# mir-group/nequip

Hardware: NVIDIA H100
Metric: atom-steps/sec (energy+forces) (higher is better)
Workload: dtype f32

## Files before the change

### nequip_b200/csrc/nqb_gemm.cu

```cuda
#include <cuda_runtime.h>
#include <stdint.h>

#include "../../include/nqb.h"
#include "nqb_tc.cuh"

namespace {

constexpr int TM = 128;
constexpr int TN = 128;
constexpr int KC = 32;
constexpr int MW = 64;
constexpr int NWG = TM / MW;
constexpr int DEPTH = 2;
constexpr int RAW = DEPTH + 1;
constexpr int NLO = 2;
constexpr int BSLOTS = 4;
constexpr int SEG = 320 / KC;
constexpr int NTHREADS = NWG * 128;
constexpr int BLOCK_FLOATS = 2 * TN * KC;

struct GemmDesc {
  int64_t a_off, c_off, b_off, rs_off;
  int64_t lda, ldc, K, N;
  int64_t kchunks, ntiles, tile0, flags;
};

struct Smem {
  float b[BSLOTS][BLOCK_FLOATS];
  float araw[NWG][RAW][MW * KC];
  float alo[NWG][NLO][MW * KC];
  uint64_t b_full[BSLOTS], b_empty[BSLOTS];
};

__device__ __forceinline__ const GemmDesc* find_desc(const GemmDesc* d, int nd, int q) {
  int i = 0;
  while (i + 1 < nd && d[i + 1].tile0 <= q) ++i;
  return d + i;
}

struct Sched {
  int q, q_step, nq_total;
  int64_t m_start, m_step;
  __device__ Sched(int b, int G, int T, const int32_t* tile_ctas, int sched_ctas) {
    nq_total = T;
    if (tile_ctas != nullptr && G == sched_ctas) {
      q = T; q_step = T; m_start = 0; m_step = 1;
      for (int t = 0; t < T; ++t) {
        const int c0 = tile_ctas[2 * t], n = tile_ctas[2 * t + 1];
        if (b >= c0 && b < c0 + n) { q = t; m_start = b - c0; m_step = n; break; }
      }
    } else if (T <= G) {
      const int R = G / T;
      q = (b < T * R) ? (b % T) : T;
      q_step = T;
      m_start = b / T;
      m_step = R;
    } else {
      q = b; q_step = G; m_start = 0; m_step = 1;
    }
  }
};

struct WorkQ {
  const GemmDesc* d;
  int nt, kchunks, K, ncols;
  bool resident;
};
__device__ __forceinline__ void decode_q(const GemmDesc* descs, int ndesc, int q, WorkQ& w) {
  w.d = find_desc(descs, ndesc, q);
  w.nt = q - (int)w.d->tile0;
  w.kchunks = (int)w.d->kchunks;
  w.K = (int)w.d->K;
  w.ncols = min(TN, (int)w.d->N - w.nt * TN);
  w.resident = w.kchunks <= BSLOTS;
}

__device__ __forceinline__ void bar_wg(int wg) { asm volatile("bar.sync %0, 128;" ::"r"(1 + wg) : "memory"); }

__global__ void __launch_bounds__(NTHREADS, 1)
k_gemm3x(const GemmDesc* __restrict__ descs, int ndesc, int ntiles_total, const int32_t* __restrict__ tile_ctas,
         int sched_ctas, const float* __restrict__ a_base, const float* __restrict__ b_base, float* __restrict__ c_base,
         const float* __restrict__ rs_base, int64_t rs_ld, int64_t M) {
  extern __shared__ __align__(1024) uint8_t smem_raw[];
  Smem& S = *reinterpret_cast<Smem*>(smem_raw);
  const int tid = threadIdx.x, wg = tid >> 7, warp = (tid >> 5) & 3, lane = tid & 31;
  const int64_t mtiles = (M + TM - 1) / TM;

  if (tid == 0) {
    for (int s = 0; s < BSLOTS; ++s) { mbar_init(&S.b_full[s], 1); mbar_init(&S.b_empty[s], NWG * 4); }
    fence_barrier_init();
  }
  __syncthreads();
  const Sched sch(blockIdx.x, gridDim.x, ntiles_total, tile_ctas, sched_ctas);

  const int r8 = lane & 7, kq = lane >> 3;
  const int my_off = (2 * warp) * (KC / 4 * 32) + kq * 32 + r8 * 4;
  int pq = sch.q, ph_ = 0, pnh = 1, pK = 0;
  int64_t pmt = sch.m_start, plda = 0;
  const float* pA = nullptr;
  bool pvalid = pq < sch.nq_total && sch.m_start < mtiles;
  auto open_q = [&]() {
    WorkQ w;
    decode_q(descs, ndesc, pq, w);
    pA = a_base + w.d->a_off;
    plda = w.d->lda;
    pK = w.K;
    pnh = w.kchunks;
  };
  if (pvalid) open_q();
  uint32_t n_issued = 0;
  auto issue = [&]() {
    if (pvalid) {
      float* dst = S.araw[wg][n_issued % RAW] + my_off;
#pragma unroll
      for (int g = 0; g < 2; ++g) {
        const int64_t m = pmt * TM + wg * MW + warp * 16 + g * 8 + r8;
#pragma unroll
        for (int kh = 0; kh < 2; ++kh) {
          const int k = ph_ * KC + (kh * 4 + kq) * 4;
          const bool in = m < M && k < pK;
          const int64_t off = in ? m * plda + k : 0;
          cp_async16(dst + g * (KC / 4 * 32) + kh * 128, pA + off, in ? 16u : 0u);
        }
      }
      if (++ph_ == pnh) {
        ph_ = 0;
        pmt += sch.m_step;
        if (pmt >= mtiles) {
          pmt = sch.m_start;
          pq += sch.q_step;
          pvalid = pq < sch.nq_total;
          if (pvalid) open_q();
        }
      }
    }
    ++n_issued;
    cp_async_commit();
  };
#pragma unroll 1
  for (int j = 0; j < DEPTH; ++j) issue();

  uint32_t bused = 0, bpar_ld = 0;
  auto load_slot = [&](int slot, const float* src, uint32_t bytes) {
    if ((bused >> slot) & 1) mbar_wait(&S.b_empty[slot], ((bpar_ld >> slot) & 1) ^ 1);
    mbar_expect_tx(&S.b_full[slot], 2 * bytes);
    bulk_g2s(S.b[slot], src, bytes, &S.b_full[slot]);
    bulk_g2s(S.b[slot] + TN * KC, src + TN * KC, bytes, &S.b_full[slot]);
    bused |= 1u << slot;
    bpar_ld ^= 1u << slot;
  };
  uint32_t bpar = 0;

  constexpr uint32_t SBO = (KC / 4) * 128, LBO = 128;
  constexpr uint32_t A_STAGE = (MW * KC * sizeof(float)) >> 4;
  constexpr uint32_t B_SLOT = (BLOCK_FLOATS * sizeof(float)) >> 4, B_LO = (TN * KC * sizeof(float)) >> 4;
  const uint64_t dR0 = make_desc(smem_u32(S.araw[wg][0]), LBO, SBO);
  const uint64_t dL0 = make_desc(smem_u32(S.alo[wg][0]), LBO, SBO);
  const uint64_t dB0 = make_desc(smem_u32(S.b[0]), LBO, SBO);
  const int r0 = warp * 16 + (lane >> 2), c0 = 2 * (lane & 3);
  float hh[64], xx[64], acc[64];
  uint32_t i = 0;

  for (int q = sch.q; q < sch.nq_total; q += sch.q_step) {
    WorkQ w;
    decode_q(descs, ndesc, q, w);
    if (sch.m_start >= mtiles) continue;
    const GemmDesc* d = w.d;
    const int nseg = (w.kchunks + SEG - 1) / SEG;
    const int64_t nmt = (mtiles - 1 - sch.m_start) / sch.m_step + 1;
    const int64_t nload = w.resident ? w.kchunks : nmt * w.kchunks;
    const uint32_t bytes = (uint32_t)TN * KC * sizeof(float);
    const float* B = b_base + d->b_off + (int64_t)w.nt * w.kchunks * BLOCK_FLOATS;
    if (tid == 0)
      for (int64_t c = 0; c < min((int64_t)BSLOTS, nload); ++c) load_slot((int)c, B + (c % w.kchunks) * BLOCK_FLOATS, bytes);
    int64_t x = 0;
    const bool reduce = (d->flags & 5) != 0, skipz = (d->flags & 2) != 0;
    const int64_t ldc = d->ldc;
    float* C = c_base + d->c_off + (int64_t)w.nt * TN;
    bool first_mt = true;
    for (int64_t mt = sch.m_start; mt < mtiles; mt += sch.m_step) {
      for (int seg = 0; seg < nseg; ++seg) {
        const int h1 = min(w.kchunks, (seg + 1) * SEG);
        for (int h = seg * SEG; h < h1; ++h, ++i) {
          cp_async_wait<DEPTH - 1>();
          const float* raw = S.araw[wg][i % RAW] + my_off;
          float* lo = S.alo[wg][i % NLO] + my_off;
#pragma unroll
          for (int g = 0; g < 2; ++g)
#pragma unroll
            for (int kh = 0; kh < 2; ++kh) {
              const float4 t = *reinterpret_cast<const float4*>(raw + g * (KC / 4 * 32) + kh * 128);
              *reinterpret_cast<float4*>(lo + g * (KC / 4 * 32) + kh * 128) =
                  make_float4(tf32_lo(t.x), tf32_lo(t.y), tf32_lo(t.z), tf32_lo(t.w));
            }
          fence_proxy_async();
          bar_wg(wg);
          uint32_t slot;
          if (w.resident) {
            slot = h;
            if (first_mt) { mbar_wait(&S.b_full[slot], (bpar >> slot) & 1); bpar ^= 1u << slot; }
          } else {
            slot = (uint32_t)(x % BSLOTS);
            mbar_wait(&S.b_full[slot], (bpar >> slot) & 1);
            bpar ^= 1u << slot;
          }
          const uint64_t a_hi = dR0 + (uint64_t)((i % RAW) * A_STAGE), a_lo = dL0 + (uint64_t)((i % NLO) * A_STAGE);
          const uint64_t b_hi = dB0 + (uint64_t)(slot * B_SLOT), b_lo = b_hi + B_LO;
          const uint32_t fresh = (h == seg * SEG);
          wgmma_fence();
#pragma unroll
          for (int ks = 0; ks < KC / 8; ++ks) wgmma_tf32_m64n128(hh, a_hi + ks * 16, b_hi + ks * 16, !(fresh && ks == 0));
#pragma unroll
          for (int ks = 0; ks < KC / 8; ++ks) wgmma_tf32_m64n128(xx, a_lo + ks * 16, b_hi + ks * 16, !(fresh && ks == 0));
#pragma unroll
          for (int ks = 0; ks < KC / 8; ++ks) wgmma_tf32_m64n128(xx, a_hi + ks * 16, b_lo + ks * 16, 1u);
          wgmma_commit();
          wgmma_wait<0>();
          if (!w.resident) {
            if (lane == 0) mbar_arrive(&S.b_empty[slot]);
            if (tid == 0 && x + BSLOTS < nload) load_slot(slot, B + ((x + BSLOTS) % w.kchunks) * BLOCK_FLOATS, bytes);
            ++x;
          }
          issue();
        }
        if (seg + 1 < nseg) {
#pragma unroll
          for (int j = 0; j < 64; ++j) acc[j] = (seg == 0 ? 0.f : acc[j]) + (hh[j] + xx[j]);
        } else {
#pragma unroll
          for (int j = 0; j < 64; ++j) hh[j] = (seg == 0) ? hh[j] + xx[j] : acc[j] + (hh[j] + xx[j]);
        }
      }
      const int64_t m0 = mt * TM + wg * MW + r0;
#pragma unroll
      for (int half = 0; half < 2; ++half) {
        const int64_t m = m0 + half * 8;
        float rs = 1.0f;
        if (d->rs_off >= 0) rs = (m < M) ? __ldg(rs_base + d->rs_off * rs_ld + m) : 0.f;
        if (m >= M || (skipz && rs == 0.f)) continue;
        float* crow = C + m * ldc + c0;
#pragma unroll
        for (int j = 0; j < TN / 8; ++j) {
          if (j * 8 + c0 < w.ncols) {
            const float v0 = hh[4 * j + 2 * half] * rs, v1 = hh[4 * j + 2 * half + 1] * rs;
            if (reduce)
              asm volatile("red.global.add.v2.f32 [%0], {%1, %2};" ::"l"(crow + j * 8), "f"(v0), "f"(v1) : "memory");
            else
              *reinterpret_cast<float2*>(crow + j * 8) = make_float2(v0, v1);
          }
        }
      }
      first_mt = false;
    }
    if (w.resident && lane == 0)
      for (int c = 0; c < w.kchunks; ++c) mbar_arrive(&S.b_empty[c]);
  }
  cp_async_wait<0>();
}

__global__ void k_gemm_prepare(const float* __restrict__ B, int64_t ldb, int K, int N, int transposed, float scale,
                               float* __restrict__ out, int kchunks, int ntiles) {
  const int64_t total = (int64_t)ntiles * kchunks * TN * KC;
  for (int64_t idx = (int64_t)blockIdx.x * blockDim.x + threadIdx.x; idx < total; idx += (int64_t)gridDim.x * blockDim.x) {
    const int kk = (int)(idx % KC);
    const int nn = (int)((idx / KC) % TN);
    const int64_t blk = idx / (KC * TN);
    const int c = (int)(blk % kchunks), j = (int)(blk / kchunks);
    const int k = c * KC + kk, n = j * TN + nn;
    float v = 0.f;
    if (k < K && n < N) v = (transposed ? B[(int64_t)n * ldb + k] : B[(int64_t)k * ldb + n]) * scale;
    const float hi = tf32_rn(v), lo = v - hi;
    float* tile = out + blk * BLOCK_FLOATS;
    const int off = canon_off(nn, kk, KC / 4);
    tile[off] = hi;
    tile[TN * KC + off] = lo;
  }
}

}

extern "C" int nqb_set_error(const char* msg);
extern "C" void nqb_count_launch(void);

static int gemm_device() {
  int dev = 0;
  cudaGetDevice(&dev);
  return dev & 63;
}
static int gemm_sm_count() {
  static int n[64] = {0};
  const int dev = gemm_device();
  if (n[dev] == 0) {
    cudaDeviceGetAttribute(&n[dev], cudaDevAttrMultiProcessorCount, dev);
    if (n[dev] <= 0) n[dev] = 132;
  }
  return n[dev];
}

extern "C" int64_t nqb_gemm_prepared_floats(int K, int N) {
  const int64_t kchunks = (K + KC - 1) / KC, ntiles = (N + TN - 1) / TN;
  return kchunks * ntiles * BLOCK_FLOATS;
}

extern "C" int nqb_gemm_prepare(const float* B, int64_t ldb, int K, int N, int transposed, float scale, float* prepared,
                                nqb_stream_t st) {
  if (!B || !prepared) return nqb_set_error("nqb_gemm_prepare: null pointer");
  if (K <= 0 || N <= 0) return nqb_set_error("nqb_gemm_prepare: bad shape");
  const int kchunks = (K + KC - 1) / KC, ntiles = (N + TN - 1) / TN;
  const int64_t total = (int64_t)ntiles * kchunks * TN * KC;
  int blocks = (int)((total + 255) / 256);
  if (blocks > 4096) blocks = 4096;
  k_gemm_prepare<<<blocks, 256, 0, (cudaStream_t)st>>>(B, ldb, K, N, transposed, scale, prepared, kchunks, ntiles);
  nqb_count_launch();
  cudaError_t e = cudaGetLastError();
  if (e != cudaSuccess) return nqb_set_error(cudaGetErrorString(e));
  return 0;
}

extern "C" int nqb_gemm_grouped(const void* descs_dev, int ndesc, int ntiles_total, const int32_t* tile_ctas_dev,
                                int sched_ctas, const float* a_base, const float* prepared_base, float* c_base,
                                const float* rowscale_base, int64_t rs_ld, int64_t M, nqb_stream_t st) {
  if (ndesc <= 0 || ntiles_total <= 0) return nqb_set_error("nqb_gemm_grouped: empty problem list");
  if (M < 0) return nqb_set_error("nqb_gemm_grouped: negative M");
  if (M == 0) return 0;
  if (!descs_dev || !a_base || !prepared_base || !c_base) return nqb_set_error("nqb_gemm_grouped: null pointer");
  static bool attr_set[64] = {false};
  const int dev = gemm_device();
  if (!attr_set[dev]) {
    cudaError_t e = cudaFuncSetAttribute(k_gemm3x, cudaFuncAttributeMaxDynamicSharedMemorySize, (int)sizeof(Smem) + 1024);
    if (e != cudaSuccess) return nqb_set_error(cudaGetErrorString(e));
    attr_set[dev] = true;
  }
  const int64_t nwork = ((M + TM - 1) / TM) * (int64_t)ntiles_total;
  int grid = (int)(nwork < gemm_sm_count() ? nwork : gemm_sm_count());
  if (tile_ctas_dev != nullptr && sched_ctas > 0 && sched_ctas <= gemm_sm_count()) grid = sched_ctas;
  else tile_ctas_dev = nullptr;
  k_gemm3x<<<grid, NTHREADS, sizeof(Smem) + 1024, (cudaStream_t)st>>>((const GemmDesc*)descs_dev, ndesc, ntiles_total, tile_ctas_dev, sched_ctas, a_base,
                                                                 prepared_base, c_base, rowscale_base, rs_ld, M);
  nqb_count_launch();
  cudaError_t e = cudaGetLastError();
  if (e != cudaSuccess) return nqb_set_error(cudaGetErrorString(e));
  return 0;
}
```

### nequip_b200/csrc/nqb_tc.cuh

```cuda
#pragma once
#define NQB_TC_HELPERS 1
#include <cuda_runtime.h>
#include <stdint.h>

namespace {

__device__ __forceinline__ uint32_t smem_u32(const void* p) { return (uint32_t)__cvta_generic_to_shared(p); }

__device__ __forceinline__ void mbar_init(uint64_t* bar, uint32_t count) {
  asm volatile("mbarrier.init.shared::cta.b64 [%0], %1;" ::"r"(smem_u32(bar)), "r"(count));
}
__device__ __forceinline__ void mbar_arrive(uint64_t* bar) {
  asm volatile("mbarrier.arrive.shared::cta.b64 _, [%0];" ::"r"(smem_u32(bar)) : "memory");
}
__device__ __forceinline__ void mbar_expect_tx(uint64_t* bar, uint32_t bytes) {
  asm volatile("mbarrier.arrive.expect_tx.shared::cta.b64 _, [%0], %1;" ::"r"(smem_u32(bar)), "r"(bytes) : "memory");
}
__device__ __forceinline__ void mbar_wait(uint64_t* bar, uint32_t parity) {
  asm volatile(
      "{\n\t"
      ".reg .pred p;\n\t"
      "WAIT_%=:\n\t"
      "mbarrier.try_wait.parity.shared::cta.b64 p, [%0], %1;\n\t"
      "@p bra DONE_%=;\n\t"
      "bra WAIT_%=;\n\t"
      "DONE_%=:\n\t"
      "}" ::"r"(smem_u32(bar)), "r"(parity) : "memory");
}
__device__ __forceinline__ void fence_barrier_init() { asm volatile("fence.mbarrier_init.release.cluster;" ::: "memory"); }
__device__ __forceinline__ void fence_proxy_async() { asm volatile("fence.proxy.async.shared::cta;" ::: "memory"); }
__device__ __forceinline__ void bulk_g2s(void* dst, const void* src, uint32_t bytes, uint64_t* bar) {
  asm volatile("cp.async.bulk.shared::cluster.global.mbarrier::complete_tx::bytes [%0], [%1], %2, [%3];" ::"r"(smem_u32(dst)),
               "l"(src), "r"(bytes), "r"(smem_u32(bar))
               : "memory");
}

__device__ __forceinline__ float4 ldg_stream(const float* p) {
  float4 v;
  asm volatile("ld.global.nc.L1::no_allocate.v4.f32 {%0, %1, %2, %3}, [%4];" : "=f"(v.x), "=f"(v.y), "=f"(v.z), "=f"(v.w) : "l"(p));
  return v;
}
__device__ __forceinline__ void cp_async16(void* dst, const void* src, uint32_t src_bytes) {
  asm volatile("cp.async.cg.shared.global [%0], [%1], 16, %2;" ::"r"(smem_u32(dst)), "l"(src), "r"(src_bytes) : "memory");
}
__device__ __forceinline__ void cp_async_commit() { asm volatile("cp.async.commit_group;" ::: "memory"); }
template <int N>
__device__ __forceinline__ void cp_async_wait() { asm volatile("cp.async.wait_group %0;" ::"n"(N) : "memory"); }
__device__ __forceinline__ float tf32_rn(float a) {
  uint32_t r;
  asm("cvt.rna.tf32.f32 %0, %1;" : "=r"(r) : "f"(a));
  return __uint_as_float(r);
}
__device__ __forceinline__ float tf32_lo(float a) {
  const float hi = __uint_as_float(__float_as_uint(a) & 0xffffe000u);
  return tf32_rn(a - hi);
}
__device__ __forceinline__ void bulk_s2g(void* dst, const void* src, uint32_t bytes) {
  asm volatile("cp.async.bulk.global.shared::cta.bulk_group [%0], [%1], %2;" ::"l"(dst), "r"(smem_u32(src)), "r"(bytes)
               : "memory");
}
__device__ __forceinline__ void bulk_s2g_add(float* dst, const float* src, uint32_t bytes) {
  asm volatile("cp.reduce.async.bulk.global.shared::cta.bulk_group.add.f32 [%0], [%1], %2;" ::"l"(dst),
               "r"(smem_u32(src)), "r"(bytes)
               : "memory");
}
__device__ __forceinline__ void bulk_commit() { asm volatile("cp.async.bulk.commit_group;" ::: "memory"); }
__device__ __forceinline__ void bulk_wait_read0() { asm volatile("cp.async.bulk.wait_group.read 0;" ::: "memory"); }
__device__ __forceinline__ void bulk_wait_all() { asm volatile("cp.async.bulk.wait_group 0;" ::: "memory"); }
__device__ __forceinline__ uint64_t make_desc(uint32_t saddr, uint32_t lbo_bytes, uint32_t sbo_bytes) {
  uint64_t d = 0;
  d |= (uint64_t)((saddr >> 4) & 0x3FFF);
  d |= (uint64_t)((lbo_bytes >> 4) & 0x3FFF) << 16;
  d |= (uint64_t)((sbo_bytes >> 4) & 0x3FFF) << 32;
  return d;
}
__device__ __forceinline__ void wgmma_fence() { asm volatile("wgmma.fence.sync.aligned;" ::: "memory"); }
__device__ __forceinline__ void wgmma_commit() { asm volatile("wgmma.commit_group.sync.aligned;" ::: "memory"); }
template <int N>
__device__ __forceinline__ void wgmma_wait() { asm volatile("wgmma.wait_group.sync.aligned %0;" ::"n"(N) : "memory"); }
__device__ __forceinline__ void wgmma_tf32_m64n128(float* d, uint64_t desc_a, uint64_t desc_b, uint32_t accumulate) {
  asm volatile(
      "{\n\t"
      ".reg .pred p;\n\t"
      "setp.ne.b32 p, %66, 0;\n\t"
      "wgmma.mma_async.sync.aligned.m64n128k8.f32.tf32.tf32 "
      "{%0, %1, %2, %3, %4, %5, %6, %7, %8, %9, %10, %11, %12, %13, %14, %15, %16, %17, %18, %19, %20, %21, %22, %23, %24, %25, %26, %27, %28, %29, %30, %31, %32, %33, %34, %35, %36, %37, %38, %39, %40, %41, %42, %43, %44, %45, %46, %47, %48, %49, %50, %51, %52, %53, %54, %55, %56, %57, %58, %59, %60, %61, %62, %63}, "
      "%64, %65, p, 1, 1;\n\t"
      "}"
      : "+f"(d[0]), "+f"(d[1]), "+f"(d[2]), "+f"(d[3]), "+f"(d[4]), "+f"(d[5]), "+f"(d[6]), "+f"(d[7]),
        "+f"(d[8]), "+f"(d[9]), "+f"(d[10]), "+f"(d[11]), "+f"(d[12]), "+f"(d[13]), "+f"(d[14]), "+f"(d[15]),
        "+f"(d[16]), "+f"(d[17]), "+f"(d[18]), "+f"(d[19]), "+f"(d[20]), "+f"(d[21]), "+f"(d[22]), "+f"(d[23]),
        "+f"(d[24]), "+f"(d[25]), "+f"(d[26]), "+f"(d[27]), "+f"(d[28]), "+f"(d[29]), "+f"(d[30]), "+f"(d[31]),
        "+f"(d[32]), "+f"(d[33]), "+f"(d[34]), "+f"(d[35]), "+f"(d[36]), "+f"(d[37]), "+f"(d[38]), "+f"(d[39]),
        "+f"(d[40]), "+f"(d[41]), "+f"(d[42]), "+f"(d[43]), "+f"(d[44]), "+f"(d[45]), "+f"(d[46]), "+f"(d[47]),
        "+f"(d[48]), "+f"(d[49]), "+f"(d[50]), "+f"(d[51]), "+f"(d[52]), "+f"(d[53]), "+f"(d[54]), "+f"(d[55]),
        "+f"(d[56]), "+f"(d[57]), "+f"(d[58]), "+f"(d[59]), "+f"(d[60]), "+f"(d[61]), "+f"(d[62]), "+f"(d[63])
      : "l"(desc_a), "l"(desc_b), "r"(accumulate));
}

__device__ __forceinline__ void wgmma_tf32_m64n64(float* d, uint64_t desc_a, uint64_t desc_b, uint32_t accumulate) {
  asm volatile(
      "{\n\t"
      ".reg .pred p;\n\t"
      "setp.ne.b32 p, %34, 0;\n\t"
      "wgmma.mma_async.sync.aligned.m64n64k8.f32.tf32.tf32 "
      "{%0, %1, %2, %3, %4, %5, %6, %7, %8, %9, %10, %11, %12, %13, %14, %15, %16, %17, %18, %19, %20, %21, %22, %23, %24, %25, %26, %27, %28, %29, %30, %31}, "
      "%32, %33, p, 1, 1;\n\t"
      "}"
      : "+f"(d[0]), "+f"(d[1]), "+f"(d[2]), "+f"(d[3]), "+f"(d[4]), "+f"(d[5]), "+f"(d[6]), "+f"(d[7]),
        "+f"(d[8]), "+f"(d[9]), "+f"(d[10]), "+f"(d[11]), "+f"(d[12]), "+f"(d[13]), "+f"(d[14]), "+f"(d[15]),
        "+f"(d[16]), "+f"(d[17]), "+f"(d[18]), "+f"(d[19]), "+f"(d[20]), "+f"(d[21]), "+f"(d[22]), "+f"(d[23]),
        "+f"(d[24]), "+f"(d[25]), "+f"(d[26]), "+f"(d[27]), "+f"(d[28]), "+f"(d[29]), "+f"(d[30]), "+f"(d[31])
      : "l"(desc_a), "l"(desc_b), "r"(accumulate));
}

__device__ __forceinline__ float2 fma2_rn(float2 a, float2 b, float2 c) {
  return make_float2(__fmaf_rn(a.x, b.x, c.x), __fmaf_rn(a.y, b.y, c.y));
}
__device__ __forceinline__ float2 fmul2_rn(float2 a, float2 b) { return make_float2(__fmul_rn(a.x, b.x), __fmul_rn(a.y, b.y)); }

__device__ __forceinline__ float silu_f(float x) { return x / (1.0f + expf(-x)); }

__device__ __forceinline__ int canon_off(int row, int k, int kgroups) {
  return (row >> 3) * (kgroups * 32) + (k >> 2) * 32 + (row & 7) * 4 + (k & 3);
}


}
```

Before: 361,800.

## Warp-specialize 3xTF32 GEMM with producer warpgroup and register-sourced A fragments

Restructures the 3xTF32 WGMMA GEMM into a warp-specialized kernel. A dedicated producer warpgroup with fewer registers streams A tiles via cp.async with mbarrier completion and B tiles via bulk copies. The two consumer warpgroups get more registers, split A into hi/lo TF32 parts in registers, and issue register-sourced wgmma with one group in flight, so the lo-part smem round trip and the per-chunk wait are gone. Segment partial sums move to shared memory, and a named-barrier handoff staggers the two consumers. This adds barrier complexity and shared-memory pressure, with a risk of hangs if the parity bookkeeping is wrong.

Result: faster. 450,700 (median of 6 runs) (+24.6%).

```diff
diff --git a/nequip_b200/csrc/nqb_gemm.cu b/nequip_b200/csrc/nqb_gemm.cu
--- a/nequip_b200/csrc/nqb_gemm.cu
+++ b/nequip_b200/csrc/nqb_gemm.cu
@@ -11,13 +11,13 @@
 constexpr int KC = 32;
 constexpr int MW = 64;
 constexpr int NWG = TM / MW;
-constexpr int DEPTH = 2;
-constexpr int RAW = DEPTH + 1;
-constexpr int NLO = 2;
+constexpr int ASLOTS = 2;
 constexpr int BSLOTS = 4;
 constexpr int SEG = 320 / KC;
-constexpr int NTHREADS = NWG * 128;
+constexpr int NTHREADS = (NWG + 1) * 128;
 constexpr int BLOCK_FLOATS = 2 * TN * KC;
+constexpr int PRODUCER_REGS = 56, CONSUMER_REGS = 224;
+constexpr int BAR_TURN = 1;
 
 struct GemmDesc {
   int64_t a_off, c_off, b_off, rs_off;
@@ -27,9 +27,10 @@
 
 struct Smem {
   float b[BSLOTS][BLOCK_FLOATS];
-  float araw[NWG][RAW][MW * KC];
-  float alo[NWG][NLO][MW * KC];
+  float acc[NWG][MW * TN];
+  float a[NWG][ASLOTS][MW * KC];
   uint64_t b_full[BSLOTS], b_empty[BSLOTS];
+  uint64_t a_full[NWG][ASLOTS], a_empty[NWG][ASLOTS];
 };
 
 __device__ __forceinline__ const GemmDesc* find_desc(const GemmDesc* d, int nd, int q) {
@@ -75,163 +76,157 @@
   w.resident = w.kchunks <= BSLOTS;
 }
 
-__device__ __forceinline__ void bar_wg(int wg) { asm volatile("bar.sync %0, 128;" ::"r"(1 + wg) : "memory"); }
-
-__global__ void __launch_bounds__(NTHREADS, 1)
-k_gemm3x(const GemmDesc* __restrict__ descs, int ndesc, int ntiles_total, const int32_t* __restrict__ tile_ctas,
-         int sched_ctas, const float* __restrict__ a_base, const float* __restrict__ b_base, float* __restrict__ c_base,
-         const float* __restrict__ rs_base, int64_t rs_ld, int64_t M) {
-  extern __shared__ __align__(1024) uint8_t smem_raw[];
-  Smem& S = *reinterpret_cast<Smem*>(smem_raw);
-  const int tid = threadIdx.x, wg = tid >> 7, warp = (tid >> 5) & 3, lane = tid & 31;
-  const int64_t mtiles = (M + TM - 1) / TM;
-
-  if (tid == 0) {
-    for (int s = 0; s < BSLOTS; ++s) { mbar_init(&S.b_full[s], 1); mbar_init(&S.b_empty[s], NWG * 4); }
-    fence_barrier_init();
-  }
-  __syncthreads();
-  const Sched sch(blockIdx.x, gridDim.x, ntiles_total, tile_ctas, sched_ctas);
-
-  const int r8 = lane & 7, kq = lane >> 3;
-  const int my_off = (2 * warp) * (KC / 4 * 32) + kq * 32 + r8 * 4;
-  int pq = sch.q, ph_ = 0, pnh = 1, pK = 0;
-  int64_t pmt = sch.m_start, plda = 0;
-  const float* pA = nullptr;
-  bool pvalid = pq < sch.nq_total && sch.m_start < mtiles;
-  auto open_q = [&]() {
-    WorkQ w;
-    decode_q(descs, ndesc, pq, w);
-    pA = a_base + w.d->a_off;
-    plda = w.d->lda;
-    pK = w.K;
-    pnh = w.kchunks;
-  };
-  if (pvalid) open_q();
-  uint32_t n_issued = 0;
-  auto issue = [&]() {
-    if (pvalid) {
-      float* dst = S.araw[wg][n_issued % RAW] + my_off;
-#pragma unroll
-      for (int g = 0; g < 2; ++g) {
-        const int64_t m = pmt * TM + wg * MW + warp * 16 + g * 8 + r8;
-#pragma unroll
-        for (int kh = 0; kh < 2; ++kh) {
-          const int k = ph_ * KC + (kh * 4 + kq) * 4;
-          const bool in = m < M && k < pK;
-          const int64_t off = in ? m * plda + k : 0;
-          cp_async16(dst + g * (KC / 4 * 32) + kh * 128, pA + off, in ? 16u : 0u);
-        }
-      }
-      if (++ph_ == pnh) {
-        ph_ = 0;
-        pmt += sch.m_step;
-        if (pmt >= mtiles) {
-          pmt = sch.m_start;
-          pq += sch.q_step;
-          pvalid = pq < sch.nq_total;
-          if (pvalid) open_q();
-        }
-      }
-    }
-    ++n_issued;
-    cp_async_commit();
-  };
-#pragma unroll 1
-  for (int j = 0; j < DEPTH; ++j) issue();
-
-  uint32_t bused = 0, bpar_ld = 0;
-  auto load_slot = [&](int slot, const float* src, uint32_t bytes) {
-    if ((bused >> slot) & 1) mbar_wait(&S.b_empty[slot], ((bpar_ld >> slot) & 1) ^ 1);
-    mbar_expect_tx(&S.b_full[slot], 2 * bytes);
-    bulk_g2s(S.b[slot], src, bytes, &S.b_full[slot]);
-    bulk_g2s(S.b[slot] + TN * KC, src + TN * KC, bytes, &S.b_full[slot]);
-    bused |= 1u << slot;
-    bpar_ld ^= 1u << slot;
-  };
-  uint32_t bpar = 0;
-
-  constexpr uint32_t SBO = (KC / 4) * 128, LBO = 128;
-  constexpr uint32_t A_STAGE = (MW * KC * sizeof(float)) >> 4;
-  constexpr uint32_t B_SLOT = (BLOCK_FLOATS * sizeof(float)) >> 4, B_LO = (TN * KC * sizeof(float)) >> 4;
-  const uint64_t dR0 = make_desc(smem_u32(S.araw[wg][0]), LBO, SBO);
-  const uint64_t dL0 = make_desc(smem_u32(S.alo[wg][0]), LBO, SBO);
-  const uint64_t dB0 = make_desc(smem_u32(S.b[0]), LBO, SBO);
-  const int r0 = warp * 16 + (lane >> 2), c0 = 2 * (lane & 3);
-  float hh[64], xx[64], acc[64];
-  uint32_t i = 0;
-
-  for (int q = sch.q; q < sch.nq_total; q += sch.q_step) {
+__device__ __forceinline__ void produce_a(Smem& S, int c, int lane, const Sched& sch, const GemmDesc* descs, int ndesc,
+                                          const float* a_base, int64_t M, int64_t mtiles) {
+  const int p = lane & 7, r0 = lane >> 3;
+  uint32_t n = 0;
+  for (int q = sch.q; q < sch.nq_total && sch.m_start < mtiles; q += sch.q_step) {
     WorkQ w;
     decode_q(descs, ndesc, q, w);
-    if (sch.m_start >= mtiles) continue;
-    const GemmDesc* d = w.d;
-    const int nseg = (w.kchunks + SEG - 1) / SEG;
+    const float* A = a_base + w.d->a_off;
+    const int64_t lda = w.d->lda;
+    for (int64_t mt = sch.m_start; mt < mtiles; mt += sch.m_step) {
+      for (int h = 0; h < w.kchunks; ++h, ++n) {
+        const uint32_t s = n % ASLOTS;
+        if (n >= ASLOTS) mbar_wait(&S.a_empty[c][s], ((n / ASLOTS) - 1) & 1);
+        float* dst = S.a[c][s] + r0 * KC;
+        const int k = h * KC + 4 * p;
+        const bool kin = k < w.K;
+        int64_t m = mt * TM + c * MW + r0;
+#pragma unroll 4
+        for (int j = 0; j < MW / 4; ++j, m += 4) {
+          const bool in = kin && m < M;
+          cp_async16(dst + 4 * j * KC + 4 * (p ^ (r0 + 4 * (j & 1))), in ? A + m * lda + k : A, in ? 16u : 0u);
+        }
+        cp_async_mbar_arrive(&S.a_full[c][s]);
+      }
+    }
+  }
+  cp_async_wait<0>();
+}
+
+__device__ __forceinline__ void produce_b(Smem& S, const Sched& sch, const GemmDesc* descs, int ndesc,
+                                          const float* b_base, int64_t mtiles) {
+  uint32_t bused = 0, bpar_ld = 0;
+  constexpr uint32_t bytes = (uint32_t)TN * KC * sizeof(float);
+  for (int q = sch.q; q < sch.nq_total && sch.m_start < mtiles; q += sch.q_step) {
+    WorkQ w;
+    decode_q(descs, ndesc, q, w);
     const int64_t nmt = (mtiles - 1 - sch.m_start) / sch.m_step + 1;
     const int64_t nload = w.resident ? w.kchunks : nmt * w.kchunks;
-    const uint32_t bytes = (uint32_t)TN * KC * sizeof(float);
-    const float* B = b_base + d->b_off + (int64_t)w.nt * w.kchunks * BLOCK_FLOATS;
-    if (tid == 0)
-      for (int64_t c = 0; c < min((int64_t)BSLOTS, nload); ++c) load_slot((int)c, B + (c % w.kchunks) * BLOCK_FLOATS, bytes);
-    int64_t x = 0;
+    const float* B = b_base + w.d->b_off + (int64_t)w.nt * w.kchunks * BLOCK_FLOATS;
+    for (int64_t x = 0; x < nload; ++x) {
+      const int slot = (int)(x % BSLOTS);
+      if ((bused >> slot) & 1) mbar_wait(&S.b_empty[slot], ((bpar_ld >> slot) & 1) ^ 1);
+      const float* src = B + (x % w.kchunks) * BLOCK_FLOATS;
+      mbar_expect_tx(&S.b_full[slot], 2 * bytes);
+      bulk_g2s(S.b[slot], src, bytes, &S.b_full[slot]);
+      bulk_g2s(S.b[slot] + TN * KC, src + TN * KC, bytes, &S.b_full[slot]);
+      bused |= 1u << slot;
+      bpar_ld ^= 1u << slot;
+    }
+  }
+}
+
+__device__ __forceinline__ void consume(Smem& S, int c, int tid, const Sched& sch, const GemmDesc* descs, int ndesc,
+                                        float* c_base, const float* rs_base, int64_t rs_ld, int64_t M, int64_t mtiles) {
+  const int warp = (tid >> 5) & 3, lane = tid & 31, ltid = tid & 127;
+  const int g = lane >> 2, t = lane & 3;
+  const int r0 = warp * 16 + g, c0 = 2 * t;
+  const float* a_frag = S.a[c][0] + r0 * KC + t;
+  float* acc = S.acc[c] + ltid;
+
+  constexpr uint32_t SBO = (KC / 4) * 128, LBO = 128;
+  constexpr uint32_t B_SLOT = (BLOCK_FLOATS * sizeof(float)) >> 4, B_LO = (TN * KC * sizeof(float)) >> 4;
+  const uint64_t dB0 = make_desc(smem_u32(S.b[0]), LBO, SBO);
+  float hh[64], xx[64];
+  uint32_t ra0[32], ra1[32];
+  uint32_t na = 0;
+  uint32_t bpar = 0;
+  bool turn_owed = false;
+
+  for (int q = sch.q; q < sch.nq_total && sch.m_start < mtiles; q += sch.q_step) {
+    WorkQ w;
+    decode_q(descs, ndesc, q, w);
+    const GemmDesc* d = w.d;
+    const int kc = w.kchunks;
     const bool reduce = (d->flags & 5) != 0, skipz = (d->flags & 2) != 0;
     const int64_t ldc = d->ldc;
     float* C = c_base + d->c_off + (int64_t)w.nt * TN;
+    int64_t x = 0;
+    int held = -1;
     bool first_mt = true;
+    auto release_b = [&](int slot) {
+      if (lane == 0) mbar_arrive(&S.b_empty[slot]);
+    };
+    auto step = [&](uint32_t(&ra)[32], int h) {
+      const uint32_t s = na % ASLOTS;
+      mbar_wait(&S.a_full[c][s], (na / ASLOTS) & 1);
+      const float* src = a_frag + s * (MW * KC);
+#pragma unroll
+      for (int ks = 0; ks < KC / 8; ++ks)
+#pragma unroll
+        for (int e = 0; e < 4; ++e) {
+          const float v = src[(e & 1) * 8 * KC + 4 * ((2 * ks + (e >> 1)) ^ g)];
+          const float hi = __uint_as_float(__float_as_uint(v) & 0xffffe000u);
+          ra[4 * ks + e] = __float_as_uint(hi);
+          ra[16 + 4 * ks + e] = __float_as_uint(tf32_rn(v - hi));
+        }
+      __syncwarp();
+      if (lane == 0) mbar_arrive(&S.a_empty[c][s]);
+      ++na;
+      uint32_t slot;
+      if (w.resident) {
+        slot = h;
+        if (first_mt) { mbar_wait(&S.b_full[slot], (bpar >> slot) & 1); bpar ^= 1u << slot; }
+        if (h == 0 && (c == 1 || turn_owed)) { named_bar_sync(BAR_TURN + c, NWG * 128); turn_owed = false; }
+      } else {
+        slot = (uint32_t)(x % BSLOTS);
+        mbar_wait(&S.b_full[slot], (bpar >> slot) & 1);
+        bpar ^= 1u << slot;
+        ++x;
+      }
+      const uint64_t b_hi = dB0 + (uint64_t)(slot * B_SLOT), b_lo = b_hi + B_LO;
+      const uint32_t fresh = (h % SEG == 0);
+      wgmma_fence();
+#pragma unroll
+      for (int ks = 0; ks < KC / 8; ++ks) wgmma_tf32_m64n128_rs(hh, ra + 4 * ks, b_hi + ks * 16, !(fresh && ks == 0));
+#pragma unroll
+      for (int ks = 0; ks < KC / 8; ++ks) wgmma_tf32_m64n128_rs(xx, ra + 16 + 4 * ks, b_hi + ks * 16, !(fresh && ks == 0));
+#pragma unroll
+      for (int ks = 0; ks < KC / 8; ++ks) wgmma_tf32_m64n128_rs(xx, ra + 4 * ks, b_lo + ks * 16, 1u);
+      wgmma_commit();
+      if (w.resident && h == kc - 1) {
+        named_bar_arrive(BAR_TURN + (c ^ 1), NWG * 128);
+        if (c == 0) turn_owed = true;
+      }
+      if ((h + 1) % SEG != 0 || h + 1 == kc) {
+        wgmma_wait<1>();
+        if (held >= 0) release_b(held);
+        held = w.resident ? -1 : (int)slot;
+        return;
+      }
+      wgmma_wait<0>();
+      if (held >= 0) release_b(held);
+      if (!w.resident) release_b(slot);
+      held = -1;
+      const int seg = h / SEG;
+#pragma unroll
+      for (int j = 0; j < 64; ++j) acc[j * 128] = (seg == 0 ? 0.f : acc[j * 128]) + (hh[j] + xx[j]);
+    };
+
     for (int64_t mt = sch.m_start; mt < mtiles; mt += sch.m_step) {
-      for (int seg = 0; seg < nseg; ++seg) {
-        const int h1 = min(w.kchunks, (seg + 1) * SEG);
-        for (int h = seg * SEG; h < h1; ++h, ++i) {
-          cp_async_wait<DEPTH - 1>();
-          const float* raw = S.araw[wg][i % RAW] + my_off;
-          float* lo = S.alo[wg][i % NLO] + my_off;
-#pragma unroll
-          for (int g = 0; g < 2; ++g)
-#pragma unroll
-            for (int kh = 0; kh < 2; ++kh) {
-              const float4 t = *reinterpret_cast<const float4*>(raw + g * (KC / 4 * 32) + kh * 128);
-              *reinterpret_cast<float4*>(lo + g * (KC / 4 * 32) + kh * 128) =
-                  make_float4(tf32_lo(t.x), tf32_lo(t.y), tf32_lo(t.z), tf32_lo(t.w));
-            }
-          fence_proxy_async();
-          bar_wg(wg);
-          uint32_t slot;
-          if (w.resident) {
-            slot = h;
-            if (first_mt) { mbar_wait(&S.b_full[slot], (bpar >> slot) & 1); bpar ^= 1u << slot; }
-          } else {
-            slot = (uint32_t)(x % BSLOTS);
-            mbar_wait(&S.b_full[slot], (bpar >> slot) & 1);
-            bpar ^= 1u << slot;
-          }
-          const uint64_t a_hi = dR0 + (uint64_t)((i % RAW) * A_STAGE), a_lo = dL0 + (uint64_t)((i % NLO) * A_STAGE);
-          const uint64_t b_hi = dB0 + (uint64_t)(slot * B_SLOT), b_lo = b_hi + B_LO;
-          const uint32_t fresh = (h == seg * SEG);
-          wgmma_fence();
-#pragma unroll
-          for (int ks = 0; ks < KC / 8; ++ks) wgmma_tf32_m64n128(hh, a_hi + ks * 16, b_hi + ks * 16, !(fresh && ks == 0));
-#pragma unroll
-          for (int ks = 0; ks < KC / 8; ++ks) wgmma_tf32_m64n128(xx, a_lo + ks * 16, b_hi + ks * 16, !(fresh && ks == 0));
-#pragma unroll
-          for (int ks = 0; ks < KC / 8; ++ks) wgmma_tf32_m64n128(xx, a_hi + ks * 16, b_lo + ks * 16, 1u);
-          wgmma_commit();
-          wgmma_wait<0>();
-          if (!w.resident) {
-            if (lane == 0) mbar_arrive(&S.b_empty[slot]);
-            if (tid == 0 && x + BSLOTS < nload) load_slot(slot, B + ((x + BSLOTS) % w.kchunks) * BLOCK_FLOATS, bytes);
-            ++x;
-          }
-          issue();
-        }
-        if (seg + 1 < nseg) {
-#pragma unroll
-          for (int j = 0; j < 64; ++j) acc[j] = (seg == 0 ? 0.f : acc[j]) + (hh[j] + xx[j]);
-        } else {
-#pragma unroll
-          for (int j = 0; j < 64; ++j) hh[j] = (seg == 0) ? hh[j] + xx[j] : acc[j] + (hh[j] + xx[j]);
-        }
-      }
-      const int64_t m0 = mt * TM + wg * MW + r0;
+      for (int h = 0; h < kc; h += 2) {
+        step(ra0, h);
+        if (h + 1 < kc) step(ra1, h + 1);
+      }
+      wgmma_wait<0>();
+      if (held >= 0) release_b(held);
+      held = -1;
+      const int seg = (kc - 1) / SEG;
+#pragma unroll
+      for (int j = 0; j < 64; ++j) hh[j] = (seg == 0) ? hh[j] + xx[j] : acc[j * 128] + (hh[j] + xx[j]);
+      const int64_t m0 = mt * TM + c * MW + r0;
 #pragma unroll
       for (int half = 0; half < 2; ++half) {
         const int64_t m = m0 + half * 8;
@@ -252,10 +247,38 @@
       }
       first_mt = false;
     }
-    if (w.resident && lane == 0)
-      for (int c = 0; c < w.kchunks; ++c) mbar_arrive(&S.b_empty[c]);
-  }
-  cp_async_wait<0>();
+    if (w.resident)
+      for (int s = 0; s < kc; ++s) release_b(s);
+  }
+  if (turn_owed) named_bar_sync(BAR_TURN, NWG * 128);
+}
+
+__global__ void __launch_bounds__(NTHREADS, 1)
+k_gemm3x(const GemmDesc* __restrict__ descs, int ndesc, int ntiles_total, const int32_t* __restrict__ tile_ctas,
+         int sched_ctas, const float* __restrict__ a_base, const float* __restrict__ b_base, float* __restrict__ c_base,
+         const float* __restrict__ rs_base, int64_t rs_ld, int64_t M) {
+  extern __shared__ __align__(1024) uint8_t smem_raw[];
+  Smem& S = *reinterpret_cast<Smem*>(smem_raw);
+  const int tid = threadIdx.x, wg = tid >> 7, warp = (tid >> 5) & 3, lane = tid & 31;
+  const int64_t mtiles = (M + TM - 1) / TM;
+
+  if (tid == 0) {
+    for (int s = 0; s < BSLOTS; ++s) { mbar_init(&S.b_full[s], 1); mbar_init(&S.b_empty[s], NWG * 4); }
+    for (int c = 0; c < NWG; ++c)
+      for (int s = 0; s < ASLOTS; ++s) { mbar_init(&S.a_full[c][s], 32); mbar_init(&S.a_empty[c][s], 4); }
+    fence_barrier_init();
+  }
+  __syncthreads();
+  if (wg == NWG) {
+    setmaxnreg_dec<PRODUCER_REGS>();
+    const Sched sch(blockIdx.x, gridDim.x, ntiles_total, tile_ctas, sched_ctas);
+    if (warp < NWG) produce_a(S, warp, lane, sch, descs, ndesc, a_base, M, mtiles);
+    else if (warp == NWG && lane == 0) produce_b(S, sch, descs, ndesc, b_base, mtiles);
+    return;
+  }
+  setmaxnreg_inc<CONSUMER_REGS>();
+  const Sched sch(blockIdx.x, gridDim.x, ntiles_total, tile_ctas, sched_ctas);
+  consume(S, wg, tid, sch, descs, ndesc, c_base, rs_base, rs_ld, M, mtiles);
 }
 
 __global__ void k_gemm_prepare(const float* __restrict__ B, int64_t ldb, int K, int N, int transposed, float scale,
diff --git a/nequip_b200/csrc/nqb_tc.cuh b/nequip_b200/csrc/nqb_tc.cuh
--- a/nequip_b200/csrc/nqb_tc.cuh
+++ b/nequip_b200/csrc/nqb_tc.cuh
@@ -98,6 +98,40 @@
       : "l"(desc_a), "l"(desc_b), "r"(accumulate));
 }
 
+__device__ __forceinline__ void wgmma_tf32_m64n128_rs(float* d, const uint32_t* a, uint64_t desc_b, uint32_t accumulate) {
+  asm volatile(
+      "{\n\t"
+      ".reg .pred p;\n\t"
+      "setp.ne.b32 p, %69, 0;\n\t"
+      "wgmma.mma_async.sync.aligned.m64n128k8.f32.tf32.tf32 "
+      "{%0, %1, %2, %3, %4, %5, %6, %7, %8, %9, %10, %11, %12, %13, %14, %15, %16, %17, %18, %19, %20, %21, %22, %23, %24, %25, %26, %27, %28, %29, %30, %31, %32, %33, %34, %35, %36, %37, %38, %39, %40, %41, %42, %43, %44, %45, %46, %47, %48, %49, %50, %51, %52, %53, %54, %55, %56, %57, %58, %59, %60, %61, %62, %63}, "
+      "{%64, %65, %66, %67}, %68, p, 1, 1;\n\t"
+      "}"
+      : "+f"(d[0]), "+f"(d[1]), "+f"(d[2]), "+f"(d[3]), "+f"(d[4]), "+f"(d[5]), "+f"(d[6]), "+f"(d[7]),
+        "+f"(d[8]), "+f"(d[9]), "+f"(d[10]), "+f"(d[11]), "+f"(d[12]), "+f"(d[13]), "+f"(d[14]), "+f"(d[15]),
+        "+f"(d[16]), "+f"(d[17]), "+f"(d[18]), "+f"(d[19]), "+f"(d[20]), "+f"(d[21]), "+f"(d[22]), "+f"(d[23]),
+        "+f"(d[24]), "+f"(d[25]), "+f"(d[26]), "+f"(d[27]), "+f"(d[28]), "+f"(d[29]), "+f"(d[30]), "+f"(d[31]),
+        "+f"(d[32]), "+f"(d[33]), "+f"(d[34]), "+f"(d[35]), "+f"(d[36]), "+f"(d[37]), "+f"(d[38]), "+f"(d[39]),
+        "+f"(d[40]), "+f"(d[41]), "+f"(d[42]), "+f"(d[43]), "+f"(d[44]), "+f"(d[45]), "+f"(d[46]), "+f"(d[47]),
+        "+f"(d[48]), "+f"(d[49]), "+f"(d[50]), "+f"(d[51]), "+f"(d[52]), "+f"(d[53]), "+f"(d[54]), "+f"(d[55]),
+        "+f"(d[56]), "+f"(d[57]), "+f"(d[58]), "+f"(d[59]), "+f"(d[60]), "+f"(d[61]), "+f"(d[62]), "+f"(d[63])
+      : "r"(a[0]), "r"(a[1]), "r"(a[2]), "r"(a[3]), "l"(desc_b), "r"(accumulate));
+}
+
+__device__ __forceinline__ void cp_async_mbar_arrive(uint64_t* bar) {
+  asm volatile("cp.async.mbarrier.arrive.noinc.shared::cta.b64 [%0];" ::"r"(smem_u32(bar)) : "memory");
+}
+template <int N>
+__device__ __forceinline__ void setmaxnreg_dec() { asm volatile("setmaxnreg.dec.sync.aligned.u32 %0;" ::"n"(N)); }
+template <int N>
+__device__ __forceinline__ void setmaxnreg_inc() { asm volatile("setmaxnreg.inc.sync.aligned.u32 %0;" ::"n"(N)); }
+__device__ __forceinline__ void named_bar_sync(int id, int nthreads) {
+  asm volatile("bar.sync %0, %1;" ::"r"(id), "r"(nthreads) : "memory");
+}
+__device__ __forceinline__ void named_bar_arrive(int id, int nthreads) {
+  asm volatile("bar.arrive %0, %1;" ::"r"(id), "r"(nthreads) : "memory");
+}
+
 __device__ __forceinline__ void wgmma_tf32_m64n64(float* d, uint64_t desc_a, uint64_t desc_b, uint32_t accumulate) {
   asm volatile(
       "{\n\t"
```
